# Samleo8/RadarSLAMPy

Measured on AMD Instinct MI355X. Metric: radar scan-pairs/sec (400x3768 polar), higher is better.
Workload: dtype u8/f32/f64

## Files before the change

### radarslampy_amd/csrc/retrack.hip

```cpp
#include "roam_internal.h"
#include "doh_common.h"
#include "blobprune.h"
#include "npsort_wave.h"
#include "retrack.h"
#include <algorithm>

#define KS ROAM_MAX_FEATURES
#define CART_CENTER 1012.0
#define M_PER_PX 0.0864
#define TWO_PI 6.283185307179586476925286766559

__global__ __launch_bounds__(256) void rt_collect_kernel(const roam_lane_result *__restrict__ res, const int32_t *__restrict__ scan_idx,
                                                         int B, int force_all, int32_t *__restrict__ rt_lane,
                                                         int32_t *__restrict__ rt_scan, int32_t *__restrict__ rt_n)
{
    __shared__ int sh[8];
    __shared__ int base_s;
    const int t = threadIdx.x;
    if (t == 0) base_s = 0;
    __syncthreads();
    for (int b0 = 0; b0 < B; b0 += 256) {
        const int b = b0 + t;
        const int f = (b < B && (force_all || (res[b].flags & 4))) ? 1 : 0;
        const int lane = t & 63, w = t >> 6;
        int inc = f;
#pragma unroll
        for (int d = 1; d < 64; d <<= 1) { int n = __shfl_up(inc, d); if (lane >= d) inc += n; }
        if (lane == 63) sh[w] = inc;
        __syncthreads();
        int off = base_s, tot = 0;
        for (int i = 0; i < 4; i++) { if (i < w) off += sh[i]; tot += sh[i]; }
        if (f) { rt_lane[off + inc - 1] = b; rt_scan[off + inc - 1] = scan_idx[b]; }
        __syncthreads();
        if (t == 0) base_s += tot;
        __syncthreads();
    }
    if (t == 0) *rt_n = base_s;
}

__device__ __forceinline__ float rt_code_to_f32(uint32_t k) { return (float)__dmul_rn((double)k, 1.0 / 255.0); }

#define RI_MIN_DETECTIONS RT_TWO_PASS_SLOTS
__device__ __forceinline__ bool rt_one_sweep(const RtArgs &a, int first) { return a.W <= 2048 && *a.rt_n - first >= RI_MIN_DETECTIONS; }

struct __attribute__((packed)) RtU16 { uint16_t v; };
struct __attribute__((packed)) RtU32 { uint32_t v; };
__device__ __forceinline__ float rt_pixel(uint32_t m, const uint8_t *__restrict__ p, int rows, int cols, int stride, const float *lut)
{
    const int ix = m & 4095, iy = (m >> 12) & 1023;
    if (ix >= cols) return 0.f;
    const float wx1 = __fmul_rn((float)((m >> 22) & 31), 1.f / 32.f), wx0 = __fsub_rn(1.f, wx1);
    const float wy1 = __fmul_rn((float)(m >> 27), 1.f / 32.f), wy0 = __fsub_rn(1.f, wy1);
    int r0 = iy - 1, r1 = iy;
    if (r0 < 0) r0 += rows; else if (r0 >= rows) r0 -= rows;
    if (r1 >= rows) r1 -= rows;
    const uint8_t *q0 = p + r0 * stride + ix, *q1 = p + r1 * stride + ix;
    const bool i1 = ix + 1 < cols;
    const int back = i1 ? 0 : 1, sh = back * 8;
    const uint32_t w0 = reinterpret_cast<const RtU16 *>(q0 - back)->v >> sh, w1 = reinterpret_cast<const RtU16 *>(q1 - back)->v >> sh;
    const float s00 = lut[w0 & 255], s01 = i1 ? lut[w0 >> 8] : 0.f;
    const float s10 = lut[w1 & 255], s11 = i1 ? lut[w1 >> 8] : 0.f;
    float v = __fmul_rn(s00, __fmul_rn(wy0, wx0));
    v = __fadd_rn(v, __fmul_rn(s01, __fmul_rn(wy0, wx1)));
    v = __fadd_rn(v, __fmul_rn(s10, __fmul_rn(wy1, wx0)));
    v = __fadd_rn(v, __fmul_rn(s11, __fmul_rn(wy1, wx1)));
    return v;
}

#define RT_TWO_PASS_Z 8
#define RC_BAND 64
#define RC_Q 16
__global__ __launch_bounds__(256) void rt_integ_cols_kernel(RtArgs a, int first, int P)
{
    const int nls = rt_one_sweep(a, first) ? 0 : min(min(RT_TWO_PASS_SLOTS, P), *a.rt_n - first);
    if ((int)blockIdx.z >= nls) return;
    __shared__ double tot[4][64];
    __shared__ float lut[256];
    __shared__ int last_s;
    lut[threadIdx.x] = rt_code_to_f32(threadIdx.x);
    const int lane = threadIdx.x & 63, q = threadIdx.x >> 6;
    const int c = blockIdx.x * 64 + lane, W = a.W, band = blockIdx.y, nb = (W + RC_BAND - 1) / RC_BAND;
    for (int ls = blockIdx.z; ls < nls; ls += (int)gridDim.z) {
    const int slot = first + ls;
    const uint8_t *p = a.pool + (int64_t)a.rt_scan[slot] * a.rec_bytes + a.payload_off;
    double *S = a.S + (int64_t)ls * a.SP * W;
    const int rows = a.rows, cols = a.cols, stride = a.stride;
    const int r0 = band * RC_BAND + q * RC_Q;
    uint32_t m[RC_Q];
#pragma unroll
    for (int k = 0; k < RC_Q; k++) m[k] = (c < W && r0 + k < W) ? a.map[(int64_t)(r0 + k) * W + c] : 0xfffu;
    __syncthreads();
    float v[RC_Q];
#pragma unroll
    for (int k = 0; k < RC_Q; k++) v[k] = rt_pixel(m[k], p, rows, cols, stride, lut);
    double s[RC_Q], acc = 0;
#pragma unroll
    for (int k = 0; k < RC_Q; k++) { acc = __dadd_rn(acc, (double)v[k]); s[k] = acc; }
    tot[q][lane] = acc;
    __syncthreads();
    double base = 0;
    for (int j = 0; j < q; j++) base = __dadd_rn(base, tot[j][lane]);
    if (c < W) {
#pragma unroll
        for (int k = 0; k < RC_Q; k++)
            if (r0 + k < W) S[(int64_t)(r0 + k) * a.SP + c] = __dadd_rn(base, s[k]);
        if (q == 3) __hip_atomic_store(a.colT + ((int64_t)ls * nb + band) * W + c, __dadd_rn(base, acc), __ATOMIC_RELAXED, __HIP_MEMORY_SCOPE_AGENT);
    }
    asm volatile("s_waitcnt vmcnt(0)" ::: "memory");
    __syncthreads();
    if (threadIdx.x == 0) last_s = atomicAdd(a.col_done + ls * 64 + (int)blockIdx.x, 1) == nb - 1;
    __syncthreads();
    if (last_s) {
    if (q == 0 && c < W) {
        double *T = a.colT + (int64_t)ls * nb * W + c;
        double run = 0.0;
        for (int b0 = 0; b0 < nb; b0 += 32) {
            double tv[32];
#pragma unroll
            for (int j = 0; j < 32; j++) tv[j] = b0 + j < nb ? __hip_atomic_load(T + (int64_t)(b0 + j) * W, __ATOMIC_RELAXED, __HIP_MEMORY_SCOPE_AGENT) : 0.0;
#pragma unroll
            for (int j = 0; j < 32; j++)
                if (b0 + j < nb) { T[(int64_t)(b0 + j) * W] = run; run = __dadd_rn(run, tv[j]); }
        }
    }
    if (threadIdx.x == 0) a.col_done[ls * 64 + (int)blockIdx.x] = 0;
    }
    __syncthreads();
    }
}

#define RR_DEPTH 4
#define RR_ROWS 16
#define RR_COLS 256
__global__ __launch_bounds__(256) void rt_integ_rows_kernel(RtArgs a, int first, int P)
{
    static_assert(RC_BAND % RR_ROWS == 0, "the rows of a workgroup lie in one band of the column pass");
    __shared__ __align__(16) double tile[RR_ROWS][RR_COLS + 2];
    const int nls = rt_one_sweep(a, first) ? 0 : min(min(RT_TWO_PASS_SLOTS, P), *a.rt_n - first);
    if ((int)blockIdx.y >= nls) return;
    const int W = a.W, H = a.W, nb = (W + RC_BAND - 1) / RC_BAND;
    const int r0 = blockIdx.x * RR_ROWS;
    for (int ls = blockIdx.y; ls < nls; ls += (int)gridDim.y) {
    double *S = a.S + (int64_t)ls * a.SP * W;
    const double *T = a.colT + ((int64_t)ls * nb + r0 / RC_BAND) * W;
    const int lc = 2 * (threadIdx.x & 127), lr = threadIdx.x >> 7;
    const int ntiles = (W + RR_COLS - 1) / RR_COLS;
    double2 reg[RR_DEPTH][8], off[RR_DEPTH];
    const int ce = (W - 1) & ~1;
    auto fetch = [&](double2 (&x)[8], double2 &o, int i) {
        const int c = i * RR_COLS + lc;
        o.x = T[min(c, W - 1)];
        o.y = T[min(c + 1, W - 1)];
#pragma unroll
        for (int k = 0; k < 8; k++) x[k] = *reinterpret_cast<const double2 *>(S + (int64_t)min(r0 + 2 * k + lr, H - 1) * a.SP + min(c, ce));
    };
#pragma unroll
    for (int d = 0; d < RR_DEPTH; d++) fetch(reg[d], off[d], min(d, ntiles - 1));
    double acc = 0;
    auto step = [&](double2 (&x)[8], double2 &o, int i) {
        const int c = i * RR_COLS + lc;
#pragma unroll
        for (int k = 0; k < 8; k++) {
            const bool rin = r0 + 2 * k + lr < H;
            *reinterpret_cast<double2 *>(&tile[2 * k + lr][lc]) =
                make_double2(rin && c < W ? __dadd_rn(x[k].x, o.x) : 0.0, rin && c + 1 < W ? __dadd_rn(x[k].y, o.y) : 0.0);
        }
        fetch(x, o, min(i + RR_DEPTH, ntiles - 1));
        __syncthreads();
#ifndef RR_NOCHAIN
        if (threadIdx.x < RR_ROWS) {
            double2 *row = reinterpret_cast<double2 *>(tile[threadIdx.x]);
            double2 y[8], z[8];
#pragma unroll
            for (int j = 0; j < 8; j++) y[j] = row[j];
            for (int j0 = 0; j0 < RR_COLS / 2; j0 += 16) {
#pragma unroll
                for (int j = 0; j < 8; j++) z[j] = row[j0 + 8 + j];
#pragma unroll
                for (int j = 0; j < 8; j++) { acc = __dadd_rn(acc, y[j].x); y[j].x = acc; acc = __dadd_rn(acc, y[j].y); y[j].y = acc; }
#pragma unroll
                for (int j = 0; j < 8; j++) row[j0 + j] = y[j];
                const int jn = min(j0 + 16, RR_COLS / 2 - 8);
#pragma unroll
                for (int j = 0; j < 8; j++) y[j] = row[jn + j];
#pragma unroll
                for (int j = 0; j < 8; j++) { acc = __dadd_rn(acc, z[j].x); z[j].x = acc; acc = __dadd_rn(acc, z[j].y); z[j].y = acc; }
#pragma unroll
                for (int j = 0; j < 8; j++) row[j0 + 8 + j] = z[j];
            }
        }
#endif
        __syncthreads();
#ifndef RR_NOSTORE
#pragma unroll
        for (int k = 0; k < 8; k++) {
            const int r = r0 + 2 * k + lr;
            const double2 t2 = *reinterpret_cast<const double2 *>(&tile[2 * k + lr][lc]);
            if (r < H && c + 1 < W) *reinterpret_cast<double2 *>(S + (int64_t)r * a.SP + c) = t2;
            else if (r < H && c < W) S[(int64_t)r * a.SP + c] = t2.x;
        }
#endif
    };
    int i0 = 0;
    for (; i0 + RR_DEPTH <= ntiles; i0 += RR_DEPTH) {
#pragma unroll
        for (int d = 0; d < RR_DEPTH; d++) step(reg[d], off[d], i0 + d);
    }
#pragma unroll
    for (int d = 0; d < RR_DEPTH - 1; d++)
        if (i0 + d < ntiles) step(reg[d], off[d], i0 + d);
    __syncthreads();
    }
}

#ifndef RI_ROWS
#define RI_ROWS 16
#endif
#ifndef RI_WAVES
#define RI_WAVES 4
#endif
#define RI_GROUPS (2048 / (64 * RI_WAVES))
#ifndef RI_LDS_PAD
#define RI_LDS_PAD 0
#endif
#ifndef RI_PHASE_SKIP
#define RI_PHASE_SKIP 1
#endif
#define RI_PHL_MAX 1024
#ifndef RI_BD
#define RI_BD 4
#endif
#define RI_TP 66
#ifndef RI_SINGLE_BUF
#define RI_SINGLE_BUF 0
#endif
#define RI_NBUF (RI_SINGLE_BUF ? 1 : 2)
#ifndef RI_ROUND
#define RI_ROUND 0
#endif
#define RI_LDS_BYTES (RI_NBUF * RI_WAVES * RI_ROWS * RI_TP * 8 + RI_LDS_PAD)
#ifndef RI_BOX
#define RI_BOX 2560
#endif
#ifndef RI_PREFETCH
#define RI_PREFETCH 1
#endif
__global__ __launch_bounds__(64) void rt_boxtab_kernel(const uint32_t *__restrict__ map, int W, int cols, uint32_t *__restrict__ boxtab)
{
    const int H = W, lane = threadIdx.x;
    const int idx = blockIdx.x, wave = idx % RI_WAVES, g = (idx / RI_WAVES) % RI_GROUPS, band = idx / (RI_WAVES * RI_GROUPS);
    const int c = min(g * 64 * RI_WAVES + 64 * wave + lane, W - 1);
    int mnx = 0x7fffffff, mxx = -1, mny = 0x7fffffff, mxy = -1;
    for (int k = 0; k < RI_ROWS; k++) {
        const uint32_t m = map[(int64_t)min(band * RI_ROWS + k, H - 1) * W + c];
        const int ix = m & 4095, iy = (m >> 12) & 1023;
        if (ix < cols) { mnx = min(mnx, ix); mxx = max(mxx, ix); mny = min(mny, iy); mxy = max(mxy, iy); }
    }
    for (int d = 32; d >= 1; d >>= 1) {
        mnx = min(mnx, __shfl_xor(mnx, d)); mxx = max(mxx, __shfl_xor(mxx, d));
        mny = min(mny, __shfl_xor(mny, d)); mxy = max(mxy, __shfl_xor(mxy, d));
    }
    if (lane == 0) {
        boxtab[2 * idx] = mxx < 0 ? 0xffff0000u : ((uint32_t)mnx | ((uint32_t)mxx << 16));
        boxtab[2 * idx + 1] = mxx < 0 ? 0u : ((uint32_t)mny | ((uint32_t)mxy << 16));
    }
}

#ifdef RI_PROF
__device__ unsigned long long ri_prof[16];
extern "C" int roam_debug_integral_prof(unsigned long long *out, int reset)
{
    if (hipMemcpyFromSymbol(out, HIP_SYMBOL(ri_prof), sizeof(ri_prof)) != hipSuccess) return -1;
    if (reset) { unsigned long long z[16] = {0}; if (hipMemcpyToSymbol(HIP_SYMBOL(ri_prof), z, sizeof(z)) != hipSuccess) return -1; }
    return 0;
}
#define RI_P(k) { const unsigned long long tn_ = __builtin_amdgcn_s_memtime(); rip_[k] += tn_ - rit_; rit_ = tn_; }
#else
#define RI_P(k)
#endif
__global__ __launch_bounds__(64 * (RI_WAVES + 1)) void rt_integral_kernel(RtArgs a, int first, int ls0)
{
#ifdef RI_PROF
    unsigned long long rip_[8] = {0}, rit_ = __builtin_amdgcn_s_memtime();
#endif
    extern __shared__ __align__(16) double ri_lds[];
    const int ls = ls0 + (int)blockIdx.x, slot = first + ls;
    if (slot >= *a.rt_n || !rt_one_sweep(a, first) || a.fused) return;
    typedef double Tile[RI_ROWS][RI_TP];
    Tile *tiles = reinterpret_cast<Tile *>(ri_lds);
    const int W = a.W, H = a.W, t = threadIdx.x, wave = t >> 6, lane = t & 63;
    const int nbands = (H + RI_ROWS - 1) / RI_ROWS;
    __shared__ float lut[256];
    __shared__ __align__(4) uint8_t box[RI_WAVES][RI_BOX];
    __shared__ uint16_t phl[RI_PHL_MAX];
    if (t < 256) lut[t] = rt_code_to_f32(t);
#if RI_PHASE_SKIP
    const int nph = (int)a.phlist[0];
    for (int i = t; i < nph; i += (int)blockDim.x) phl[i] = (uint16_t)a.phlist[1 + i];
#else
    const int nph = nbands * RI_GROUPS;
    for (int i = t; i < nph; i += (int)blockDim.x) phl[i] = (uint16_t)((i / RI_GROUPS) | ((i % RI_GROUPS) << 8) | (((1u << RI_WAVES) - 1u) << 12));
#endif
    __syncthreads();
    auto ph_ent = [&](int i) { return i < nph ? (int)__builtin_amdgcn_readfirstlane((int)phl[i]) : 0; };
    auto ph_band = [](int e) { return e & 255; };
    auto ph_group = [](int e) { return (e >> 8) & 15; };
    if (wave < RI_WAVES) {
        const uint8_t *p = a.pool + (int64_t)a.rt_scan[slot] * a.rec_bytes + a.payload_off;
        double *S = a.S + (int64_t)ls * a.SP * W;
        const int SP = a.SP;
        const int rows = a.rows, cols = a.cols, stride = a.stride;
        double acc[RI_GROUPS];
#pragma unroll
        for (int g = 0; g < RI_GROUPS; g++) acc[g] = 0.0;
        uint32_t m[RI_ROWS];
        uint32_t ext0 = 0, ext1 = 0;
        uint32_t cur0 = 0xffff0000u, cur1 = 0;
        uint32_t raw[8];
        const int wave_u = __builtin_amdgcn_readfirstlane(wave);
        auto fetch = [&](int band, int g) {
            const int c = min(g * 64 * RI_WAVES + 64 * wave + lane, W - 1);
#pragma unroll
            for (int k = 0; k < RI_ROWS; k++) m[k] = a.map[(int64_t)min(band * RI_ROWS + k, H - 1) * W + c];
        };
        auto fetch_ext = [&](int i) {
            const uint32_t *bt = a.boxtab + 2 * (i * RI_WAVES + wave_u);
            ext0 = bt[0]; ext1 = bt[1];
        };
        struct Box { int mnx, mxx, mny, mxy, bh, bp, nrg, ncb; bool staged, inside; };
        auto geom = [&](uint32_t e0, uint32_t e1) {
            Box b;
            b.mnx = e0 & 0xffff; b.mxx = (e0 >> 16) == 0xffff ? -1 : (int)(e0 >> 16); b.mny = e1 & 0xffff; b.mxy = e1 >> 16;
            const int bw = b.mxx - b.mnx + 2;
            b.bh = b.mxy - b.mny + 2; b.bp = (bw + 3) & ~3;
            b.nrg = (b.bh + 3) >> 2; b.ncb = (b.bp + 63) >> 6;
            b.staged = b.mxx >= 0 && b.bp * b.bh <= RI_BOX && cols >= 4;
            b.inside = b.staged && b.mny >= 1 && b.mny - 1 + 4 * b.nrg <= rows && b.mnx + 64 * b.ncb <= cols;
            return b;
        };
        const int sub = lane >> 4, c4 = (lane & 15) * 4;
        auto load_pieces = [&](const Box &b, int q0) {
            const uint8_t *pl = p + (sub * stride + c4);
            const int npiece = b.nrg * b.ncb;
            int kg = (q0 / b.ncb) * 4, cb = (q0 % b.ncb) * 64;
#pragma unroll
            for (int u = 0; u < 8; u++) {
                if (q0 + u < npiece) raw[u] = reinterpret_cast<const RtU32 *>(pl + ((b.mny - 1 + kg) * stride + b.mnx + cb))->v;
                cb += 64;
                if (cb >= b.bp) { cb = 0; kg += 4; }
            }
        };
        auto store_pieces = [&](const Box &b, int q0, uint8_t *bx) {
            uint8_t *bl = bx + (sub * b.bp + c4);
            const int npiece = b.nrg * b.ncb;
            int kg = (q0 / b.ncb) * 4, cb = (q0 % b.ncb) * 64;
#pragma unroll
            for (int u = 0; u < 8; u++) {
                if (q0 + u < npiece && sub < b.bh - kg && c4 < b.bp - cb) *reinterpret_cast<uint32_t *>(bl + (kg * b.bp + cb)) = raw[u];
                cb += 64;
                if (cb >= b.bp) { cb = 0; kg += 4; }
            }
        };
        auto prefetch_box = [&]() {
            cur0 = __builtin_amdgcn_readfirstlane(ext0); cur1 = __builtin_amdgcn_readfirstlane(ext1);
#if RI_PREFETCH
            const Box b = geom(cur0, cur1);
            if (b.inside) load_pieces(b, 0);
#endif
        };
        float v[RI_ROWS];
        auto A1 = [&](int i, int e_n1, int e_n2) {
            const Box b = geom(cur0, cur1);
            const int mnx = b.mnx, mny = b.mny, bh = b.bh, bp = b.bp;
            if (b.mxx < 0) {
#pragma unroll
                for (int k = 0; k < RI_ROWS; k++) v[k] = 0.f;
            } else if (b.staged) {
                uint8_t *bx = box[wave];
                if (b.inside) {
                    const int npiece = b.nrg * b.ncb;
                    for (int q0 = 0; q0 < npiece; q0 += 8) {
                        if (q0 > 0 || !RI_PREFETCH) load_pieces(b, q0);
                        store_pieces(b, q0, bx);
                    }
                } else
                for (int kg = 0; kg < bh; kg += 4) {
                    const int kk = kg + sub;
                    int r = mny + kk - 1;
                    if (r < 0) r += rows; else if (r >= rows) r -= rows;
                    for (int cb = 0; cb < bp; cb += 64) {
                        const int cc = cb + c4;
                        if (kk < bh && cc < bp) {
                            const int x0 = mnx + cc, xl = min(x0, cols - 4), sh = 8 * (x0 - xl);
                            uint32_t rw = 0;
                            if (sh < 32) rw = reinterpret_cast<const RtU32 *>(p + r * stride + xl)->v >> sh;
                            *reinterpret_cast<uint32_t *>(bx + kk * bp + cc) = rw;
                        }
                    }
                }
#pragma unroll
                for (int k = 0; k < RI_ROWS; k++) {
                    const uint32_t mk = m[k];
                    const int ix = mk & 4095, iy = (mk >> 12) & 1023;
                    float r_ = 0.f;
                    if (ix < cols) {
                        const float wx1 = __fmul_rn((float)((mk >> 22) & 31), 1.f / 32.f), wx0 = __fsub_rn(1.f, wx1);
                        const float wy1 = __fmul_rn((float)(mk >> 27), 1.f / 32.f), wy0 = __fsub_rn(1.f, wy1);
                        const uint8_t *q = bx + (iy - mny) * bp + (ix - mnx);
#ifdef RI_TAP_VALU
                        auto dec = [](uint32_t k) { const float kf = (float)k; return __fmaf_rn(kf, 0x1.0101020000000p-8f, __fmul_rn(kf, -0x1.fdfdfe0000000p-33f)); };
                        const float s00 = dec(q[0]), s01 = dec(q[1]), s10 = dec(q[bp]), s11 = dec(q[bp + 1]);
#elif defined(RI_TAP16)
                        const uint32_t w0 = reinterpret_cast<const RtU16 *>(q)->v, w1 = reinterpret_cast<const RtU16 *>(q + bp)->v;
                        const float s00 = lut[w0 & 255], s01 = lut[w0 >> 8], s10 = lut[w1 & 255], s11 = lut[w1 >> 8];
#else
                        const float s00 = lut[q[0]], s01 = lut[q[1]], s10 = lut[q[bp]], s11 = lut[q[bp + 1]];
#endif
                        r_ = __fmul_rn(s00, __fmul_rn(wy0, wx0));
                        r_ = __fadd_rn(r_, __fmul_rn(s01, __fmul_rn(wy0, wx1)));
                        r_ = __fadd_rn(r_, __fmul_rn(s10, __fmul_rn(wy1, wx0)));
                        r_ = __fadd_rn(r_, __fmul_rn(s11, __fmul_rn(wy1, wx1)));
                    }
                    v[k] = r_;
                }
            } else {
#pragma unroll
                for (int k = 0; k < RI_ROWS; k++) v[k] = rt_pixel(m[k], p, rows, cols, stride, lut);
            }
            if (i + 1 < nph) {
                fetch(ph_band(e_n1), ph_group(e_n1));
                prefetch_box();
                if (i + 2 < nph) fetch_ext(ph_band(e_n2) * RI_GROUPS + ph_group(e_n2));
            }
        };
        int gcur = 0;
        auto A2 = [&](int i, int band, int g) {
            const int c = g * 64 * RI_WAVES + 64 * wave + lane;
            Tile &tl = tiles[(RI_SINGLE_BUF ? 0 : (i & 1)) * RI_WAVES + wave];
            {
                while (gcur != g) {
                    const double s0 = acc[0];
#pragma unroll
                    for (int q = 0; q + 1 < RI_GROUPS; q++) acc[q] = acc[q + 1];
                    acc[RI_GROUPS - 1] = s0;
                    gcur = (gcur + 1) % RI_GROUPS;
                }
                double s = acc[0];
                if (c < W) {
#pragma unroll
                    for (int k = 0; k < RI_ROWS; k++) {
                        if (band * RI_ROWS + k < H) s = __dadd_rn(s, (double)v[k]);
                        tl[k][lane] = s;
                    }
                }
#pragma unroll
                for (int q = 0; q + 1 < RI_GROUPS; q++) acc[q] = acc[q + 1];
                acc[RI_GROUPS - 1] = s;
                gcur = (gcur + 1) % RI_GROUPS;
            }
        };
        auto C = [&](int i, int e) {
            const int band = ph_band(e), g = ph_group(e);
            const int c = g * 64 * RI_WAVES + 64 * wave + lane;
            const Tile &tl = tiles[(RI_SINGLE_BUF ? 0 : (i & 1)) * RI_WAVES + wave];
            const bool wanted = ((e >> (12 + wave_u)) & 1) != 0;
            if (c < W && wanted) {
                double *q = S + (int64_t)band * RI_ROWS * SP + c;
                const int nk = min(RI_ROWS, H - band * RI_ROWS);
                if (nk == RI_ROWS) {
#pragma unroll
                    for (int k = 0; k < RI_ROWS; k++) q[(int64_t)k * SP] = tl[k][lane];
                } else
                    for (int k = 0; k < nk; k++) q[(int64_t)k * SP] = tl[k][lane];
            }
        };
        int e_m1 = 0, e_0 = ph_ent(0), e_1 = ph_ent(1), e_2 = ph_ent(2), e_3 = ph_ent(3);
        if (nph > 0) {
            fetch(ph_band(e_0), ph_group(e_0));
            fetch_ext(ph_band(e_0) * RI_GROUPS + ph_group(e_0));
            prefetch_box();
            if (nph > 1) fetch_ext(ph_band(e_1) * RI_GROUPS + ph_group(e_1));
            A1(0, e_1, e_2);
#if RI_SINGLE_BUF
#pragma unroll 1
            for (int i = 0; i < nph; i++) {
                const int e_4 = ph_ent(i + 4);
                A2(i, ph_band(e_0), ph_group(e_0));
                __syncthreads();
                if (i + 1 < nph) A1(i + 1, e_2, e_3);
                __syncthreads();
                C(i, e_0);
                e_m1 = e_0; e_0 = e_1; e_1 = e_2; e_2 = e_3; e_3 = e_4;
            }
        }
#else
            A2(0, ph_band(e_0), ph_group(e_0));
#pragma unroll 1
            for (int i = 0; i < nph; i++) {
                const int e_4 = ph_ent(i + 4);
                RI_P(0)
                __syncthreads();
                RI_P(1)
                if (i > 0) C(i - 1, e_m1);
                RI_P(2)
                if (i + 1 < nph) { A1(i + 1, e_2, e_3); RI_P(3) A2(i + 1, ph_band(e_1), ph_group(e_1)); }
                RI_P(4)
                e_m1 = e_0; e_0 = e_1; e_1 = e_2; e_2 = e_3; e_3 = e_4;
            }
        }
        __syncthreads();
        if (nph > 0) C(nph - 1, e_m1);
#endif
    } else {
        double carry = 0.0;
// ... 1341 lines not shown
```

Baseline: 53370.

## Replace serial row prefix sum with exact wave-parallel fixed-point scan

The row pass of the integral image used to run a serial chain of double adds, one thread per row over an LDS tile. It now uses a wave-parallel scan, one wave per row. The scan represents each rounding step as a pair of fixed-point integer maps composed through shuffles, so it reproduces the exact round-to-nearest-even result of the sequential double sum. When the running sum crosses a magnitude boundary it falls back and restarts from that point. This removes the long dependent add chain and the LDS tile with its barriers, at the cost of integer work, shuffles, and possible repeated passes when the exponent changes.

```diff
diff --git a/radarslampy_amd/csrc/retrack.hip b/radarslampy_amd/csrc/retrack.hip
--- a/radarslampy_amd/csrc/retrack.hip
+++ b/radarslampy_amd/csrc/retrack.hip
@@ -129,87 +129,121 @@
     }
 }
 
-#define RR_DEPTH 4
-#define RR_ROWS 16
-#define RR_COLS 256
+#define RR_ROWS 4
+#define RS_K 4
+#define RS_SPAN (64 * RS_K)
+#define RS_TOP (1ull << 53)
+struct RsMap { uint64_t d0, d1; };
+__device__ __forceinline__ RsMap rs_then(RsMap a, RsMap b)
+{
+    return {a.d0 + ((a.d0 & 1) ? b.d1 : b.d0), a.d1 + ((a.d1 & 1) ? b.d0 : b.d1)};
+}
+__device__ __forceinline__ RsMap rs_elem(uint64_t X, int sh)
+{
+    const uint64_t q = X >> sh, f = X & ((1ull << sh) - 1), half = sh ? 1ull << (sh - 1) : 0;
+    const bool up = f > half, tie = sh > 0 && f == half, odd = (q & 1) != 0;
+    return {q + ((up || (tie && odd)) ? 1 : 0), q + ((up || (tie && !odd)) ? 1 : 0)};
+}
+__device__ __forceinline__ void rs_span(const double (&x)[RS_K], double (&out)[RS_K], uint64_t &n, int &sh, int lane)
+{
+    uint64_t X[RS_K];
+#pragma unroll
+    for (int k = 0; k < RS_K; k++) X[k] = (uint64_t)__dmul_rn(x[k], 0x1p41);
+    int start = 0;
+    for (;;) {
+        const double u = ldexp(1.0, sh - 41);
+        RsMap e[RS_K];
+#pragma unroll
+        for (int k = 0; k < RS_K; k++) e[k] = RS_K * lane + k < start ? RsMap{0, 0} : rs_elem(X[k], sh);
+        RsMap f = e[0];
+#pragma unroll
+        for (int k = 1; k < RS_K; k++) f = rs_then(f, e[k]);
+#pragma unroll
+        for (int d = 1; d < 64; d <<= 1) {
+            const RsMap g = {__shfl_up(f.d0, d), __shfl_up(f.d1, d)};
+            if (lane >= d) f = rs_then(g, f);
+        }
+        RsMap ex = {__shfl_up(f.d0, 1), __shfl_up(f.d1, 1)};
+        if (lane == 0) ex = {0, 0};
+        uint64_t m = n + ((n & 1) ? ex.d1 : ex.d0), mb = 0, v[RS_K];
+        int bad = RS_K;
+#pragma unroll
+        for (int k = 0; k < RS_K; k++) {
+            const uint64_t prev = m;
+            m += (m & 1) ? e[k].d1 : e[k].d0;
+            v[k] = m;
+            if (bad == RS_K && m >= RS_TOP) { bad = k; mb = prev; }
+        }
+        const uint64_t lanes_bad = __ballot(bad < RS_K);
+        const int bl = lanes_bad ? __ffsll((unsigned long long)lanes_bad) - 1 : 64;
+#pragma unroll
+        for (int k = 0; k < RS_K; k++)
+            if (RS_K * lane + k >= start && (lane < bl || (lane == bl && k < bad))) out[k] = __dmul_rn((double)v[k], u);
+        if (!lanes_bad) { n = __shfl(m, 63); return; }
+        double s = 0.0;
+        if (lane == bl) {
+#pragma unroll
+            for (int k = 0; k < RS_K; k++)
+                if (k == bad) { s = __dadd_rn(__dmul_rn((double)mb, u), x[k]); out[k] = s; }
+        }
+        s = __shfl(s, bl);
+        start = RS_K * bl + __shfl(bad, bl) + 1;
+        sh = max(0, ilogb(s) - 11);
+        n = (uint64_t)__dmul_rn(s, ldexp(1.0, 41 - sh));
+        if (start >= RS_SPAN) return;
+    }
+}
+#define RR_DEPTH 3
 __global__ __launch_bounds__(256) void rt_integ_rows_kernel(RtArgs a, int first, int P)
 {
     static_assert(RC_BAND % RR_ROWS == 0, "the rows of a workgroup lie in one band of the column pass");
-    __shared__ __align__(16) double tile[RR_ROWS][RR_COLS + 2];
     const int nls = rt_one_sweep(a, first) ? 0 : min(min(RT_TWO_PASS_SLOTS, P), *a.rt_n - first);
     if ((int)blockIdx.y >= nls) return;
     const int W = a.W, H = a.W, nb = (W + RC_BAND - 1) / RC_BAND;
-    const int r0 = blockIdx.x * RR_ROWS;
+    const int lane = threadIdx.x & 63, r = blockIdx.x * RR_ROWS + (threadIdx.x >> 6);
+    if (r >= H) return;
+    const int nsp = (W + RS_SPAN - 1) / RS_SPAN;
     for (int ls = blockIdx.y; ls < nls; ls += (int)gridDim.y) {
-    double *S = a.S + (int64_t)ls * a.SP * W;
-    const double *T = a.colT + ((int64_t)ls * nb + r0 / RC_BAND) * W;
-    const int lc = 2 * (threadIdx.x & 127), lr = threadIdx.x >> 7;
-    const int ntiles = (W + RR_COLS - 1) / RR_COLS;
-    double2 reg[RR_DEPTH][8], off[RR_DEPTH];
-    const int ce = (W - 1) & ~1;
-    auto fetch = [&](double2 (&x)[8], double2 &o, int i) {
-        const int c = i * RR_COLS + lc;
-        o.x = T[min(c, W - 1)];
-        o.y = T[min(c + 1, W - 1)];
-#pragma unroll
-        for (int k = 0; k < 8; k++) x[k] = *reinterpret_cast<const double2 *>(S + (int64_t)min(r0 + 2 * k + lr, H - 1) * a.SP + min(c, ce));
+    double *Sr = a.S + ((int64_t)ls * W + r) * a.SP;
+    const double *T = a.colT + ((int64_t)ls * nb + r / RC_BAND) * W;
+    double2 sx[RR_DEPTH][2];
+    double tx[RR_DEPTH][RS_K];
+    auto fetch = [&](int d, int i) {
+        const int c = i * RS_SPAN + RS_K * lane, cs = c < W ? c : 0;
+        sx[d][0] = *reinterpret_cast<const double2 *>(Sr + cs);
+        sx[d][1] = *reinterpret_cast<const double2 *>(Sr + cs + 2);
+#pragma unroll
+        for (int k = 0; k < RS_K; k++) tx[d][k] = T[min(c + k, W - 1)];
     };
 #pragma unroll
-    for (int d = 0; d < RR_DEPTH; d++) fetch(reg[d], off[d], min(d, ntiles - 1));
-    double acc = 0;
-    auto step = [&](double2 (&x)[8], double2 &o, int i) {
-        const int c = i * RR_COLS + lc;
-#pragma unroll
-        for (int k = 0; k < 8; k++) {
-            const bool rin = r0 + 2 * k + lr < H;
-            *reinterpret_cast<double2 *>(&tile[2 * k + lr][lc]) =
-                make_double2(rin && c < W ? __dadd_rn(x[k].x, o.x) : 0.0, rin && c + 1 < W ? __dadd_rn(x[k].y, o.y) : 0.0);
-        }
-        fetch(x, o, min(i + RR_DEPTH, ntiles - 1));
-        __syncthreads();
-#ifndef RR_NOCHAIN
-        if (threadIdx.x < RR_ROWS) {
-            double2 *row = reinterpret_cast<double2 *>(tile[threadIdx.x]);
-            double2 y[8], z[8];
-#pragma unroll
-            for (int j = 0; j < 8; j++) y[j] = row[j];
-            for (int j0 = 0; j0 < RR_COLS / 2; j0 += 16) {
-#pragma unroll
-                for (int j = 0; j < 8; j++) z[j] = row[j0 + 8 + j];
-#pragma unroll
-                for (int j = 0; j < 8; j++) { acc = __dadd_rn(acc, y[j].x); y[j].x = acc; acc = __dadd_rn(acc, y[j].y); y[j].y = acc; }
-#pragma unroll
-                for (int j = 0; j < 8; j++) row[j0 + j] = y[j];
-                const int jn = min(j0 + 16, RR_COLS / 2 - 8);
-#pragma unroll
-                for (int j = 0; j < 8; j++) y[j] = row[jn + j];
-#pragma unroll
-                for (int j = 0; j < 8; j++) { acc = __dadd_rn(acc, z[j].x); z[j].x = acc; acc = __dadd_rn(acc, z[j].y); z[j].y = acc; }
-#pragma unroll
-                for (int j = 0; j < 8; j++) row[j0 + 8 + j] = z[j];
-            }
-        }
-#endif
-        __syncthreads();
-#ifndef RR_NOSTORE
-#pragma unroll
-        for (int k = 0; k < 8; k++) {
-            const int r = r0 + 2 * k + lr;
-            const double2 t2 = *reinterpret_cast<const double2 *>(&tile[2 * k + lr][lc]);
-            if (r < H && c + 1 < W) *reinterpret_cast<double2 *>(S + (int64_t)r * a.SP + c) = t2;
-            else if (r < H && c < W) S[(int64_t)r * a.SP + c] = t2.x;
-        }
-#endif
+    for (int d = 0; d < RR_DEPTH; d++) fetch(d, min(d, nsp - 1));
+    uint64_t n = 0;
+    int sh = 0;
+    auto step = [&](int d, int i) {
+        const int c = i * RS_SPAN + RS_K * lane;
+        const double sv[RS_K] = {sx[d][0].x, sx[d][0].y, sx[d][1].x, sx[d][1].y};
+        double x[RS_K], out[RS_K];
+#pragma unroll
+        for (int k = 0; k < RS_K; k++) x[k] = c + k < W ? __dadd_rn(sv[k], tx[d][k]) : 0.0;
+        fetch(d, min(i + RR_DEPTH, nsp - 1));
+        rs_span(x, out, n, sh, lane);
+        if (c + RS_K <= W) {
+            *reinterpret_cast<double2 *>(Sr + c) = make_double2(out[0], out[1]);
+            *reinterpret_cast<double2 *>(Sr + c + 2) = make_double2(out[2], out[3]);
+        } else {
+#pragma unroll
+            for (int k = 0; k < RS_K; k++)
+                if (c + k < W) Sr[c + k] = out[k];
+        }
     };
     int i0 = 0;
-    for (; i0 + RR_DEPTH <= ntiles; i0 += RR_DEPTH) {
-#pragma unroll
-        for (int d = 0; d < RR_DEPTH; d++) step(reg[d], off[d], i0 + d);
+    for (; i0 + RR_DEPTH <= nsp; i0 += RR_DEPTH) {
+#pragma unroll
+        for (int d = 0; d < RR_DEPTH; d++) step(d, i0 + d);
     }
 #pragma unroll
     for (int d = 0; d < RR_DEPTH - 1; d++)
-        if (i0 + d < ntiles) step(reg[d], off[d], i0 + d);
-    __syncthreads();
+        if (i0 + d < nsp) step(d, i0 + d);
     }
 }
 
```

Result: no change. 53230 (median of 2 runs) (-0.2%).
